# cvjena/mvlm

Hardware: AMD Instinct MI355X
Metric: views/sec (render+CNN+fuse) per mesh, 256x256x96 views (higher is better)
Workload: dtype f32; 1 GPU; configs[2] BU_3DFE-RGB+depth.json: 96 views @ 256x256 of one 99458-triangle textured synthetic face OBJ, 84 landmarks, 4 input channels (RGB+depth), seeded random weights; views_total=96, views_per_gpu=96, landmarks=84, in_channels=4, triangles=99458, selection_method=simple, parallelism=1 GPU, no collective

## Files before the change

### include/mvlm_hip.h

```cpp
#ifndef MVLM_HIP_H
#define MVLM_HIP_H

#include <stddef.h>
#include <stdint.h>

#ifdef __cplusplus
extern "C" {
#endif

typedef struct mvlm_ctx mvlm_ctx;
typedef struct mvlm_mesh mvlm_mesh;
typedef struct mvlm_texture mvlm_texture;

#define MVLM_IMAGE_SIZE 256
#define MVLM_CONV_DESC_INTS 12

enum { MVLM_MODE_QUANTILE = 0, MVLM_MODE_ABSOLUTE = 1 };
enum { MVLM_MAXIMA_SIMPLE = 0, MVLM_MAXIMA_MOMENT = 1 };

int mvlm_ctx_create(int device, mvlm_ctx** out);
void mvlm_ctx_destroy(mvlm_ctx* ctx);
const char* mvlm_last_error(mvlm_ctx* ctx);
int mvlm_set_stream(mvlm_ctx* ctx, void* hip_stream);
int mvlm_synchronize(mvlm_ctx* ctx);
// ... 72 lines not shown
size_t mvlm_cnn_workspace_bytes(mvlm_ctx* ctx, int batch);
int mvlm_cnn_maxima(mvlm_ctx* ctx, const float* images_dev, int n_views, const int32_t* chan_sel_host,
                    float* maxima_dev, void* workspace_dev, size_t workspace_bytes, int batch);
int mvlm_cnn_set_selection(mvlm_ctx* ctx, int method);
int mvlm_cnn_heatmaps(mvlm_ctx* ctx, const float* images_dev, int n_views, const int32_t* chan_sel_host,
                      float* heat_dev, void* workspace_dev, size_t workspace_bytes, int batch);
int mvlm_cnn_set_execution(mvlm_ctx* ctx, int graph_mode, int concurrency);
int mvlm_cnn_set_pairing(mvlm_ctx* ctx, int mode);
int mvlm_cnn_set_winograd(mvlm_ctx* ctx, int mode);
int mvlm_pack_winograd_weights(const float* w9_host, int cin_pad, int cout_pad, float* w12_host);
int mvlm_cnn_set_winograd4(mvlm_ctx* ctx, int mode);
int mvlm_pack_winograd4_weights(const float* w9_host, int cin_pad, int cout_pad, float* w18_host);
int mvlm_cnn_set_winograd4_wide(mvlm_ctx* ctx, int on);
int mvlm_conv_wino4_wide_serves(int ksize, int cin_pad, int cout_pad, int size);
int mvlm_conv_wino4_wide_launches(mvlm_ctx* ctx, int64_t* count, int reset);
int mvlm_cnn_execution_stats(mvlm_ctx* ctx, int64_t* eager_runs, int64_t* graph_captures, int64_t* graph_replays,
                             int64_t* graph_failures);
size_t mvlm_pack_fast_weights(const float* w, int cout, int cin, int cout_pad, int cin_pad, uint16_t* out);
int mvlm_cnn_load_fast(mvlm_ctx* ctx, const uint16_t* blob_host, size_t n_u16, const int64_t* slot_offsets, int n_slots);
int mvlm_cnn_set_precision(mvlm_ctx* ctx, int fast);
int mvlm_conv2d_fast(mvlm_ctx* ctx, const float* x_dev, int batch, int cin, int h, int w, const float* w_host, int cout,
                     const float* bias_host, const float* pre_scale_host, const float* pre_shift_host,
                     const float* post_scale_host, const float* post_shift_host, const float* r_dev, float* y_dev);
size_t mvlm_pack_fast_weights16(const float* w, int cout, int cin, int cout_pad, int cin_pad, uint16_t* out, float* unscale);
int mvlm_cnn_load_fast16(mvlm_ctx* ctx, const uint16_t* blob_host, size_t n_u16, const int64_t* slot_offsets,
                         const float* slot_unscale, int n_slots);
int mvlm_cnn_fast16_overflowed(mvlm_ctx* ctx, int* overflowed);
int mvlm_conv2d_fast16(mvlm_ctx* ctx, const float* x_dev, int batch, int cin, int h, int w, const float* w_host, int cout,
                       const float* bias_host, const float* pre_scale_host, const float* pre_shift_host,
                       const float* post_scale_host, const float* post_shift_host, const float* r_dev, float* y_dev);
// ... 61 lines not shown
```

### mvlm_amd/_lib.py

```python
from __future__ import annotations

import ctypes as C
import os
import subprocess
import threading
from pathlib import Path

_HERE = Path(__file__).resolve().parent
LIB_PATH = Path(os.environ["MVLM_HIP_LIB"]) if os.environ.get("MVLM_HIP_LIB") else _HERE / "lib" / "libmvlm_hip.so"
CSRC = _HERE / "csrc"

c_float_p = C.POINTER(C.c_float)
c_double_p = C.POINTER(C.c_double)
c_int32_p = C.POINTER(C.c_int32)
c_uint8_p = C.POINTER(C.c_uint8)

SIGNATURES = {
    "mvlm_ctx_create": (C.c_int, [C.c_int, C.POINTER(C.c_void_p)]),
    "mvlm_ctx_destroy": (None, [C.c_void_p]),
    "mvlm_last_error": (C.c_char_p, [C.c_void_p]),
    "mvlm_set_stream": (C.c_int, [C.c_void_p, C.c_void_p]),
    "mvlm_synchronize": (C.c_int, [C.c_void_p]),
    "mvlm_build_arch": (C.c_char_p, []),
    "mvlm_obj_read": (C.c_int, [C.c_char_p, C.POINTER(C.c_void_p), C.c_char_p, C.c_int]),
# ... 52 lines not shown
    "mvlm_cnn_workspace_bytes": (C.c_size_t, [C.c_void_p, C.c_int]),
    "mvlm_cnn_maxima": (C.c_int, [C.c_void_p, C.c_void_p, C.c_int, c_int32_p, C.c_void_p, C.c_void_p, C.c_size_t,
                                  C.c_int]),
    "mvlm_cnn_heatmaps": (C.c_int, [C.c_void_p, C.c_void_p, C.c_int, c_int32_p, C.c_void_p, C.c_void_p, C.c_size_t,
                                    C.c_int]),
    "mvlm_cnn_set_execution": (C.c_int, [C.c_void_p, C.c_int, C.c_int]),
    "mvlm_cnn_set_selection": (C.c_int, [C.c_void_p, C.c_int]),
    "mvlm_cnn_set_pairing": (C.c_int, [C.c_void_p, C.c_int]),
    "mvlm_cnn_set_winograd": (C.c_int, [C.c_void_p, C.c_int]),
    "mvlm_pack_winograd_weights": (C.c_int, [c_float_p, C.c_int, C.c_int, c_float_p]),
    "mvlm_cnn_set_winograd4": (C.c_int, [C.c_void_p, C.c_int]),
    "mvlm_pack_winograd4_weights": (C.c_int, [c_float_p, C.c_int, C.c_int, c_float_p]),
    "mvlm_cnn_set_winograd4_wide": (C.c_int, [C.c_void_p, C.c_int]),
    "mvlm_conv_wino4_wide_serves": (C.c_int, [C.c_int, C.c_int, C.c_int, C.c_int]),
    "mvlm_conv_wino4_wide_launches": (C.c_int, [C.c_void_p, C.POINTER(C.c_int64), C.c_int]),
    "mvlm_cnn_execution_stats": (C.c_int, [C.c_void_p, C.POINTER(C.c_int64), C.POINTER(C.c_int64), C.POINTER(C.c_int64),
                                          C.POINTER(C.c_int64)]),
    "mvlm_pack_fast_weights": (C.c_size_t, [c_float_p, C.c_int, C.c_int, C.c_int, C.c_int, C.POINTER(C.c_uint16)]),
    "mvlm_cnn_load_fast": (C.c_int, [C.c_void_p, C.POINTER(C.c_uint16), C.c_size_t, C.POINTER(C.c_int64), C.c_int]),
    "mvlm_cnn_set_precision": (C.c_int, [C.c_void_p, C.c_int]),
    "mvlm_pack_fast_weights16": (C.c_size_t, [c_float_p, C.c_int, C.c_int, C.c_int, C.c_int, C.POINTER(C.c_uint16), c_float_p]),
    "mvlm_cnn_load_fast16": (C.c_int, [C.c_void_p, C.POINTER(C.c_uint16), C.c_size_t, C.POINTER(C.c_int64), c_float_p, C.c_int]),
    "mvlm_cnn_fast16_overflowed": (C.c_int, [C.c_void_p, C.POINTER(C.c_int)]),
    "mvlm_conv2d_fast16": (C.c_int, [C.c_void_p, C.c_void_p, C.c_int, C.c_int, C.c_int, C.c_int, c_float_p, C.c_int, c_float_p,
                                     c_float_p, c_float_p, c_float_p, c_float_p, C.c_void_p, C.c_void_p]),
    "mvlm_conv2d_fast": (C.c_int, [C.c_void_p, C.c_void_p, C.c_int, C.c_int, C.c_int, C.c_int, c_float_p, C.c_int, c_float_p,
                                   c_float_p, c_float_p, c_float_p, c_float_p, C.c_void_p, C.c_void_p]),
    "mvlm_cnn_set_profiling": (C.c_int, [C.c_void_p, C.c_int]),
    "mvlm_cnn_get_profile": (C.c_int, [C.c_void_p, c_int32_p, c_int32_p, c_double_p, c_float_p, C.c_int]),
    "mvlm_conv_variant_name": (C.c_char_p, [C.c_int]),
# ... 140 lines not shown
```

### mvlm_amd/csrc/api.hip

```cpp
#include <atomic>
#include <cstring>

#include <memory>

#include <cmath>

#include "common.h"
#include "raster_points_math.h"
#include "raster_view_math.h"

void* mvlm_ctx::get_scratch(const char* name, size_t bytes) {
    auto& e = scratch[name];
    if (e.second >= bytes && e.first) return e.first;
    if (e.first) {
        hipStreamSynchronize(stream);
        hipFree(e.first);
        e = {nullptr, 0};
    }
    void* p = nullptr;
    const size_t want = bytes + bytes / 4 + 256;
    if (hipMalloc(&p, want) != hipSuccess) return nullptr;
    e = {p, want};
    return p;
}
// ... 19 lines not shown
    *out = ctx;
    return 0;
}

extern "C" void mvlm_ctx_destroy(mvlm_ctx* ctx) {
    if (!ctx) return;
    hipSetDevice(ctx->device);
    hipStreamSynchronize(ctx->stream);
    for (auto& kv : ctx->scratch)
        if (kv.second.first) hipFree(kv.second.first);
    if (ctx->cnn.blob) hipFree(ctx->cnn.blob);
    if (ctx->cnn.fast_blob) hipFree(ctx->cnn.fast_blob);
    if (ctx->cnn.fast16_blob) hipFree(ctx->cnn.fast16_blob);
    for (auto& ww : ctx->cnn.wino)
        if (ww.blob) hipFree(ww.blob);
    if (ctx->cnn.fast16_flag) hipFree(ctx->cnn.fast16_flag);
    if (ctx->switch_event) hipEventDestroy(ctx->switch_event);
    for (int i = 0; i < 2; ++i) {
        if (ctx->kparts_ws[i]) hipFree(ctx->kparts_ws[i]);
        if (ctx->kparts_cnt[i]) hipFree(ctx->kparts_cnt[i]);
    }
    for (auto& e : ctx->mesh_pool) {
        hipFree(e.p);
        if (e.freed) hipEventDestroy(e.freed);
    }
    for (hipEvent_t e : ctx->event_free) hipEventDestroy(e);
    for (int i = 0; i < 2; ++i) {
        if (ctx->upload_stage[i]) hipHostFree(ctx->upload_stage[i]);
        if (ctx->upload_stage_done[i]) hipEventDestroy(ctx->upload_stage_done[i]);
    }
// ... 548 lines not shown
    auto vec = [&](const float* src, int n, int n_pad) -> long {
        if (!src) return -1;
        const size_t off = push(n_pad);
        for (int i = 0; i < n; ++i) blob[off + i] = src[i];
        return long(off);
    };
    long ww_off[MVLM_WINO_FORMS_N];
    for (int f = 0; f < MVLM_WINO_FORMS_N; ++f) {
        const WinoForm& form = mvlm_wino_form(f);
        ww_off[f] = -1;
        if (!form.serves_slot(ksize, cin_pad, cout_pad)) continue;
        ww_off[f] = long(push(size_t(form.slices) * cin_pad * cout_pad));
        form.transform(blob.data() + w_off, cin_pad, cout_pad, blob.data() + ww_off[f]);
    }
    const long b_off = vec(bias_host, cout, cout_pad);
    const long ps_off = vec(pre_scale_host, cin, cin_pad), pt_off = vec(pre_shift_host, cin, cin_pad);
    const long qs_off = vec(post_scale_host, cout, cout_pad), qt_off = vec(post_shift_host, cout, cout_pad);
    auto* d = static_cast<float*>(ctx->get_scratch("conv2d.blob", blob.size() * 4));
    MVLM_REQUIRE(ctx, d, "conv2d: scratch allocation failed");
    MVLM_CHECK_HIP(ctx, hipMemcpy(d, blob.data(), blob.size() * 4, hipMemcpyHostToDevice));
    ConvArgs a;
    a.in = x_dev;
    a.in_ctot = cin;
    a.cin = cin;
    a.cin_pad = cin_pad;
    a.up_in = upsample_in;
    a.B = batch;
    a.H = h;
    a.W = w;
    a.w = d + w_off;
    for (int f = 0; f < MVLM_WINO_FORMS_N; ++f) a.*mvlm_wino_form(f).weights = ww_off[f] < 0 ? nullptr : d + ww_off[f];
    a.cout = cout;
    a.cout_pad = cout_pad;
    a.ksize = ksize;
    a.bias = b_off < 0 ? nullptr : d + b_off;
    a.pre_scale = ps_off < 0 ? nullptr : d + ps_off;
    a.pre_shift = pt_off < 0 ? nullptr : d + pt_off;
    a.post_scale = qs_off < 0 ? nullptr : d + qs_off;
    a.post_shift = qt_off < 0 ? nullptr : d + qt_off;
    a.res1 = r_dev;
    a.res1_ctot = cout;
    a.out = y_dev;
    a.out_ctot = cout;
    if (mvlm_launch_conv(ctx, a, nullptr)) return 1;
    MVLM_CHECK_HIP(ctx, hipStreamSynchronize(ctx->stream));
    return 0;
}

extern "C" int mvlm_conv_bench(mvlm_ctx* ctx, int batch, int cin, int cout, int ksize, int size, int flags, int variant,
                               int iters, float* ms_per_launch, int* variant_used) {
    MVLM_ENTER(ctx);
    MVLM_REQUIRE(ctx, batch > 0 && cin > 0 && cout > 0 && size > 0 && iters > 0 && ms_per_launch, "conv_bench: bad arguments");
    MVLM_REQUIRE(ctx, ksize == 1 || ksize == 3, "conv_bench: kernel size must be 1 or 3");
    const int cin_pad = (ksize == 1 ? (cin + 7) / 8 * 8 : (cin + 3) / 4 * 4), taps = ksize * ksize;
    const bool plain = (flags & 4) && !(flags & (1 | 2 | 8));
    const int cout_pad = (plain && (cout + 15) / 16 * 16 == 80) ? 80 : (plain && ksize == 3 && cout == 84) ? 84 : (cout + 31) / 32 * 32;
    const size_t px = size_t(batch) * size * size;
    const size_t n_w = size_t(ksize == 3 ? 18 : taps) * cin_pad * cout_pad, n_vec = size_t(cin_pad) * 2 + size_t(cout_pad) * 3;
    const size_t n_x = px * cin, n_y = px * cout;
    const size_t total = n_w + n_vec + n_x + 3 * n_y + 64;
    auto* base = static_cast<float*>(ctx->get_scratch("conv_bench", total * sizeof(float)));
    MVLM_REQUIRE(ctx, base, "conv_bench: scratch allocation failed");
    MVLM_CHECK_HIP(ctx, hipMemsetAsync(base, 0, total * sizeof(float), ctx->stream));
    float* w = base;
    float* vec = w + n_w;
    float* x = vec + (n_vec + 3) / 4 * 4;
    float* y = x + (n_x + 3) / 4 * 4;
    float* raw = y + (n_y + 3) / 4 * 4;
    float* res = raw + (n_y + 3) / 4 * 4;
    ConvArgs a;
    a.in = x;
    a.in_ctot = cin;
    a.cin = cin;
    a.cin_pad = cin_pad;
    a.B = batch;
    a.H = a.W = size;
    a.w = w;
    for (int f = 0; f < MVLM_WINO_FORMS_N; ++f)
        if (mvlm_wino_form(f).serves_slot(ksize, cin_pad, cout_pad)) a.*mvlm_wino_form(f).weights = w;
    a.cout = cout;
    a.cout_pad = cout_pad;
    a.ksize = ksize;
    if (flags & 1) {
        a.pre_scale = vec;
        a.pre_shift = vec + cin_pad;
    }
    if (flags & 4) a.bias = vec + 2 * cin_pad;
    if (flags & 8) {
        a.post_scale = vec + 2 * cin_pad + cout_pad;
        a.post_shift = vec + 2 * cin_pad + 2 * cout_pad;
    }
    if (flags & 2) {
        a.res1 = res;
        a.res1_ctot = cout;
// ... 251 lines not shown
```

### mvlm_amd/csrc/cnn_graph.hip

```cpp
#include <cstdlib>

#include "common.h"

namespace {

constexpr long CONCURRENT_MAX_PIXELS_32 = 32l * 32 * 32;

struct Tensor {
    float* p = nullptr;
    int C = 0, S = 0;
    size_t off = 0, elems = 0;
};

struct Block {
    size_t off, size;
    bool free;
    int arena;
    bool deferred;
};

struct Exec {
    mvlm_ctx* ctx;
    CnnState& st;
    int B;
// ... 104 lines not shown
        const int32_t* r = d(slot);
        if (!r[0]) return rc = ctx->fail("cnn: conv slot not present in the packed weights");
        a.in = x.p;
        a.in_ctot = x.C;
        a.in_coff = 0;
        a.cin = r[1];
        a.cout = r[2];
        a.ksize = r[3];
        a.cin_pad = r[4];
        a.cout_pad = r[5];
        a.w = blob(r[6]);
        for (int f = 0; f < MVLM_WINO_FORMS_N; ++f) {
            const CnnState::WinoWeights& ww = st.wino[f];
            a.*mvlm_wino_form(f).weights = (size_t(slot) < ww.off.size() && ww.off[size_t(slot)] >= 0) ? ww.blob + ww.off[size_t(slot)] : nullptr;
        }
        a.bias = blob(r[7]);
        a.pre_scale = blob(r[8]);
        a.pre_shift = blob(r[9]);
        a.post_scale = blob(r[10]);
        a.post_shift = blob(r[11]);
        a.B = B;
        a.H = a.W = S;
        if (x.C != a.cin) return rc = ctx->fail("cnn: channel mismatch between graph and packed weights");
        return 0;
    }
    bool runs_fast(int slot, const ConvArgs& a) const {
        const std::vector<long long>& off = st.fast == 2 ? st.fast16_off : st.fast_off;
        return st.fast && size_t(slot) < off.size() && off[size_t(slot)] >= 0 && mvlm_conv_fast_ok(a, st.fast == 2 ? 2 : 3);
    }
    int prof_begin(hipEvent_t& e0, hipEvent_t& e1) {
// ... 613 lines not shown
        st.fast_blob = nullptr;
    }
    st.fast16_off.clear();
    st.fast16_unscale.clear();
    if (st.fast16_blob) {
        (void)hipFree(st.fast16_blob);
        st.fast16_blob = nullptr;
    }
    for (CnnState::WinoWeights& ww : st.wino) {
        ww.off.clear();
        if (ww.blob) {
            (void)hipFree(ww.blob);
            ww.blob = nullptr;
        }
    }
    st.drop_graphs();
    st.desc.assign(desc_host, desc_host + size_t(n_slots) * MVLM_CONV_DESC_INTS);
    for (int s = 0; s < n_slots; ++s) {
        const int32_t* r = &st.desc[size_t(s) * MVLM_CONV_DESC_INTS];
        if (!r[0]) continue;
        MVLM_REQUIRE(ctx, r[1] > 0 && r[2] > 0 && r[3] >= 1 && r[3] <= 3, "cnn_load: bad conv shape");
        MVLM_REQUIRE(ctx, r[4] % 4 == 0 && r[4] >= r[1] && (r[5] % 16 == 0 || (r[5] == 84 && r[2] == 84 && (r[3] == 3 || r[3] == 2))) && r[5] >= r[2],
                     "cnn_load: bad padding");
        const size_t wsz = size_t(r[3]) * r[3] * r[4] * r[5];
        MVLM_REQUIRE(ctx, r[6] >= 0 && size_t(r[6]) + wsz <= n_floats, "cnn_load: weight offset out of range");
        const int offs[5] = {r[7], r[8], r[9], r[10], r[11]};
        const int lens[5] = {r[5], r[4], r[4], r[5], r[5]};
        for (int k = 0; k < 5; ++k)
            MVLM_REQUIRE(ctx, offs[k] < 0 || size_t(offs[k]) + lens[k] <= n_floats, "cnn_load: vector offset out of range");
    }
// ... 8 lines not shown
        std::vector<float> host;
        ww.off.assign(size_t(n_slots), -1);
        for (int s = 0; s < n_slots; ++s) {
            const int32_t* r = &st.desc[size_t(s) * MVLM_CONV_DESC_INTS];
            if (!r[0] || !form.serves_slot(r[3], r[4], r[5])) continue;
            const size_t off = host.size();
            host.resize(off + size_t(form.slices) * r[4] * r[5]);
            form.transform(blob_host + r[6], r[4], r[5], host.data() + off);
            ww.off[size_t(s)] = (long long)off;
        }
        if (!host.empty()) {
            MVLM_CHECK_HIP(ctx, hipMalloc(&ww.blob, host.size() * sizeof(float)));
            MVLM_CHECK_HIP(ctx, hipMemcpy(ww.blob, host.data(), host.size() * sizeof(float), hipMemcpyHostToDevice));
        }
    }
    st.n_landmarks = n_landmarks;
    st.in_channels = in_channels;
    st.loaded = true;
    return 0;
}

extern "C" size_t mvlm_cnn_workspace_bytes(mvlm_ctx* ctx, int batch) {
    std::lock_guard<std::mutex> lk(ctx->mu);
    if (!ctx->cnn.loaded || batch <= 0) return 0;
    Exec ex(ctx, batch, nullptr, 0, true);
    const int sel4[4] = {0, 0, 0, 0};
    ex.forward(nullptr, sel4, reinterpret_cast<float*>(8), 0, batch, nullptr);
    return ex.high + 256;
}

// ... 56 lines not shown
}

extern "C" int mvlm_cnn_set_winograd(mvlm_ctx* ctx, int mode) {
    return set_winograd_mode(ctx, &mvlm_ctx::conv_winograd, mode, "cnn_set_winograd: 0 never, 1 the measured table (default), 2 every layer a Winograd variant can serve");
}

extern "C" int mvlm_cnn_set_winograd4(mvlm_ctx* ctx, int mode) {
    return set_winograd_mode(ctx, &mvlm_ctx::conv_winograd4, mode, "cnn_set_winograd4: 0 never, 1 the measured table (default), 2 every layer the F(4,3) Winograd tile can serve");
}

extern "C" int mvlm_cnn_set_winograd4_wide(mvlm_ctx* ctx, int on) {
    MVLM_ENTER(ctx);
    MVLM_REQUIRE(ctx, on == 0 || on == 1, "cnn_set_winograd4_wide: 0 the 32 x 16 shape on every launch, 1 the wide shape where the output channels come in 64s (default)");
    if (on != ctx->conv_winograd4_wide) ctx->cnn.drop_graphs();
    ctx->conv_winograd4_wide = on;
    return 0;
}

extern "C" int mvlm_conv_wino4_wide_launches(mvlm_ctx* ctx, int64_t* count, int reset) {
    std::lock_guard<std::mutex> lk(ctx->mu);
    if (count) *count = ctx->conv_wino4_wide_launches;
    if (reset) ctx->conv_wino4_wide_launches = 0;
    return 0;
}

extern "C" int mvlm_cnn_execution_stats(mvlm_ctx* ctx, int64_t* eager_runs, int64_t* graph_captures,
                                        int64_t* graph_replays, int64_t* graph_failures) {
    std::lock_guard<std::mutex> lk(ctx->mu);
    const CnnState& st = ctx->cnn;
    if (eager_runs) *eager_runs = st.eager_runs;
// ... 124 lines not shown
```

### mvlm_amd/csrc/common.h

```cpp
#pragma once
#include <hip/hip_runtime.h>

#include <cstdint>
#include <cstdio>
#include <cstdlib>
#include <map>
#include <mutex>
#include <string>
#include <vector>

#include "../../include/mvlm_hip.h"
#include "jpeg_plan.h"

#define MVLM_CHECK_HIP(ctx, expr)                                                            \
    do {                                                                                     \
        hipError_t _e = (expr);                                                              \
        if (_e != hipSuccess) {                                                              \
            (ctx)->fail(std::string(#expr) + ": " + hipGetErrorString(_e));                  \
            return 1;                                                                        \
        }                                                                                    \
    } while (0)

#define MVLM_ENTER(ctx)                               \
    std::lock_guard<std::mutex> _mvlm_lock((ctx)->mu); \
// ... 24 lines not shown
__host__ __device__ inline bool argmax_better(float ov, int oi, float bv, int bi) {
    const int ok = argmax_key(ov), bk = argmax_key(bv);
    return ok > bk || (ok == bk && oi < bi);
}

struct ConvArgs {
    const float* in = nullptr;
    int in_ctot = 0, in_coff = 0;
    int cin = 0, cin_pad = 0;
    int up_in = 0;
    const float* pre_scale = nullptr;
    const float* pre_shift = nullptr;
    int B = 0, H = 0, W = 0;
    const float* w = nullptr;
    int cout = 0, cout_pad = 0, ksize = 3;
    const float* bias = nullptr;
    const float* post_scale = nullptr;
    const float* post_shift = nullptr;
    const float* res1 = nullptr;
    int res1_ctot = 0, res1_coff = 0;
    const float* res2 = nullptr;
    int res2_ctot = 0, res2_coff = 0;
    float* out_raw = nullptr;
    int raw_ctot = 0, raw_coff = 0;
    float* out = nullptr;
    int out_ctot = 0, out_coff = 0;
    int up_out = 0;
    int sub_y = 0, sub_x = 0;
    int n_par = 1;
    const float* w_par[4] = {nullptr, nullptr, nullptr, nullptr};
// ... 6 lines not shown
    float* kws = nullptr;
    unsigned* kcnt = nullptr;
    float* amax_val = nullptr;
    int* amax_idx = nullptr;
    int amax_parts = 0;
    int amax_part0 = 0;
    float* pool_out = nullptr;
    int pool_ctot = 0, pool_coff = 0;
    float fast_unscale = 1.f;
    int pool_hint = 0;
    unsigned* fast_ovf = nullptr;
    const float* w_wino4 = nullptr;
    unsigned long long* timing = nullptr;
    const float* w_wino = nullptr;
};
static_assert(sizeof(ConvArgs) == 360 && offsetof(ConvArgs, fast_ovf) == 328 && offsetof(ConvArgs, timing) == 344,
              "ConvArgs is passed to the kernels by value: moving a field changes the device code of every convolution kernel");

struct ConvProfileRec {
    int slot, variant;
    double flops;
    hipEvent_t e0, e1;
    short shape[6] = {0, 0, 0, 0, 0, 0};
};

struct ConvOverride {
    short ksize, cin_pad, cout_pad, size, kind;
    int variant;
};
struct ConvKey {
    short ksize, cin_pad, cout_pad, size, kind, batch;
};
// ... 36 lines not shown
    int graph_mode = 1;
    int concurrency = 0;
    int selection = 0;
    int pairing = 1;
    unsigned short* fast_blob = nullptr;
    std::vector<long long> fast_off;
    int fast = 0;
    unsigned short* fast16_blob = nullptr;
    std::vector<long long> fast16_off;
    std::vector<float> fast16_unscale;
    unsigned* fast16_flag = nullptr;
    struct WinoWeights {
        float* blob = nullptr;
        std::vector<long long> off;
    } wino[MVLM_WINO_FORMS_N];
    std::vector<CnnGraphEntry> graphs;
    long graph_replays = 0, graph_captures = 0, eager_runs = 0, graph_failures = 0;
    void drop_graphs() {
        for (CnnGraphEntry& g : graphs)
            if (g.exec) hipGraphExecDestroy(g.exec);
        graphs.clear();
    }
};

struct mvlm_mesh {
    float* verts = nullptr;
    float* uvs = nullptr;
    int32_t* tris = nullptr;
    uint8_t* tex = nullptr;
    uint8_t* colors = nullptr;
// ... 31 lines not shown
    const void* snap_vert_tri = nullptr;
    hipEvent_t switch_event = nullptr;
    bool track_order = false;
    bool order_recorded = false;
    std::mutex mu;
    std::string err;
    CnnState cnn;
    std::map<std::string, std::pair<void*, size_t>> scratch;
    float* kparts_ws[2] = {nullptr, nullptr};
    unsigned* kparts_cnt[2] = {nullptr, nullptr};
    int conv_force_variant = -1;
    int conv_winograd = [] { const char* e = getenv("MVLM_WINOGRAD"); return (e && e[0] >= '0' && e[0] <= '2' && !e[1]) ? e[0] - '0' : 1; }();
    int conv_winograd4 = [] { const char* e = getenv("MVLM_WINOGRAD4"); return (e && e[0] >= '0' && e[0] <= '2' && !e[1]) ? e[0] - '0' : 1; }();
    int conv_winograd4_wide = [] { const char* e = getenv("MVLM_WINOGRAD4_WIDE"); return (e && e[0] >= '0' && e[0] <= '1' && !e[1]) ? e[0] - '0' : 1; }();
    long long conv_wino4_wide_launches = 0;
    std::vector<ConvOverride> conv_overrides;
    unsigned long long conv_attr_mask = 0;
    struct KeyPlaneState {
        const void* ptr = nullptr;
        size_t cap = 0;
    };
    KeyPlaneState raster_keys_clean;
    KeyPlaneState raster_keys4_clean;
    int render_subpixel_bits = 8;
    int render_multisamples = 0;
    int render_shading = 0;
    int* render_overflow_host = nullptr;
    bool points_counting = false;
    std::vector<hipEvent_t> points_events;
    bool points_events_valid = false;
// ... 87 lines not shown
int mvlm_conv_pair_variant(const ConvArgs& a0, const ConvArgs& a1, int mode);
int mvlm_launch_conv_pair(mvlm_ctx* ctx, const ConvArgs& a0, const ConvArgs& a1, int pair_variant);
int mvlm_conv_amax_parts(int H, int W);
const char* mvlm_conv_variant_name_impl(int v);

inline int mvlm_fast_cin_pad(int cin) { return (cin + 15) / 16 * 16; }
inline int mvlm_fast_cout_pad(int cout) { return cout <= 32 ? 32 : (cout + 63) / 64 * 64; }
inline bool mvlm_fast_channels_ok(int cin, int cout) {
    return cin >= 16 && cin <= 256 && cout > 0 && cout * 8 >= mvlm_fast_cout_pad(cout) * 5;
}
bool mvlm_conv_fast_ok(const ConvArgs& a, int splits);
int mvlm_launch_conv_fast(mvlm_ctx* ctx, const ConvArgs& a, const unsigned short* wq_dev, int splits = 3, float unscale = 1.f);
constexpr int MVLM_CONV_VARIANT_WINO4 = 2048;
constexpr int MVLM_CONV_WINO4_ATTR_BIT = 41, MVLM_CONV_WINO4_WIDE_ATTR_BIT = 42, MVLM_CONV_FAST_ATTR_BIT0 = 54;
inline bool mvlm_conv_wino4_wide_shape_ok(int cout_pad, int H) { return cout_pad > 0 && cout_pad % 64 == 0 && H % 16 == 0; }
constexpr int MVLM_CONV_VARIANT_FAST = 62;
constexpr int MVLM_CONV_VARIANT_FAST16 = 61;

int mvlm_launch_landmark_view(mvlm_ctx* ctx, const mvlm_mesh* mesh, const double* rot_host, int n_views, int size,
                              const float* frames_host, const double* landmarks_host, int n_lm, float radius,
                              const uint8_t* lm_rgb_host, uint8_t* out_dev, int32_t* lm_pixels_dev);

int mvlm_launch_ray_view(mvlm_ctx* ctx, const mvlm_mesh* mesh, const double* rot_host, int n_views, int size,
                         const float* frames_host, const double* landmarks_host, int n_lm, float radius, const uint8_t* lm_rgb_host,
                         const double* starts_dev, const double* ends_dev, int n_rays, float ray_radius, const uint8_t* ray_rgb_host,
                         uint8_t* out_dev, int32_t* lm_pixels_dev, int32_t* ray_pixels_dev);

int mvlm_project_partials(mvlm_ctx* ctx, const mvlm_mesh* mesh, const double* pts_dev, int n_points, int* n_chunks_out,
                          const double** part_d_out, const int** part_t_out);

// ... 12 lines not shown
```

### mvlm_amd/csrc/conv_inst_g12.hip

```cpp
#include "conv_kernel.h"
#include "conv_variants.h"

#define X(id, name, ...) \
    int mvlm_conv_launch_##id(mvlm_ctx* ctx, const ConvArgs& a) { return launch_variant<__VA_ARGS__>(ctx, a, id); } \
    int mvlm_conv_pair_launch_##id(mvlm_ctx* ctx, const ConvArgs& a0, const ConvArgs& a1) { return launch_variant_pair<__VA_ARGS__>(ctx, a0, a1, id); }
MVLM_CONV_VARIANTS_G12(X)
#undef X
```

### mvlm_amd/csrc/conv_inst_g3.hip

```cpp
#include "conv_kernel.h"
#include "conv_variants.h"

#define X(id, name, ...) \
    int mvlm_conv_launch_##id(mvlm_ctx* ctx, const ConvArgs& a) { return launch_variant<__VA_ARGS__>(ctx, a, id); } \
    int mvlm_conv_pair_launch_##id(mvlm_ctx* ctx, const ConvArgs& a0, const ConvArgs& a1) { return launch_variant_pair<__VA_ARGS__>(ctx, a0, a1, id); }
MVLM_CONV_VARIANTS_G3(X)
#undef X
```

### mvlm_amd/csrc/conv_inst_q0.hip

```cpp
#include "conv_kernel.h"
#include "conv_variants.h"
#include "conv_wino4_wide_hold.h"

int mvlm_conv_launch_wino4_wide(mvlm_ctx* ctx, const ConvArgs& a);

static bool wide_shape_held(const ConvArgs& a) {
    const int kind = mvlm_conv_kind(a);
    for (int i = 0; i < MVLM_CONV_WINO4_WIDE_HOLD_N; ++i) {
        const ConvWino4WideHold& e = MVLM_CONV_WINO4_WIDE_HOLD[i];
        if (e.cin_pad == a.cin_pad && e.cout_pad == a.cout_pad && e.size == a.H && e.kind == kind) return true;
    }
    return false;
}

int mvlm_conv_launch_wino4(mvlm_ctx* ctx, const ConvArgs& a) {
    if (ctx->conv_winograd4_wide && mvlm_conv_wino4_wide_shape_ok(a.cout_pad, a.H) && !wide_shape_held(a)) return mvlm_conv_launch_wino4_wide(ctx, a);
    return launch_variant<MVLM_CONV_WINO4_CFG>(ctx, a, MVLM_CONV_WINO4_ATTR_BIT);
}
```

### mvlm_amd/csrc/conv_mfma.hip

```cpp
#include <algorithm>
#include <array>
#include <cstdlib>
#include <map>
#include <mutex>
#include <string>
#include <tuple>
#include <vector>

#include "common.h"
#include "conv_kernel.h"
#include "conv_variants.h"
#include "conv_tuned.h"
#include "conv_tuned_net.h"
#include "conv_pair_tuned.h"
#include "conv_tuned_wino.h"
#include "conv_tuned_wino4.h"

#define X(id, name, ...)                                         \
    int mvlm_conv_launch_##id(mvlm_ctx* ctx, const ConvArgs& a); \
    int mvlm_conv_pair_launch_##id(mvlm_ctx* ctx, const ConvArgs& a0, const ConvArgs& a1);
MVLM_CONV_VARIANTS(X)
#undef X
int mvlm_conv_launch_wino4(mvlm_ctx* ctx, const ConvArgs& a);

// ... 321 lines not shown
    MVLM_REQUIRE(ctx, v >= 0, "conv: no kernel variant for this shape");
    const VariantCode d = decode_variant(v);
    const WinoForm* form = d.row && d.row->form >= 0 ? &mvlm_wino_form(d.row->form) : nullptr;
    MVLM_REQUIRE(ctx, !form || a.*form->weights, std::string("conv: a Winograd tile needs the layer's transformed weights (") + form->pack_fn + ")");
    MVLM_REQUIRE(ctx, !a.in2 || v == 0, "conv: a second input tensor needs the 128-channel 8x32 tile (ask mvlm_conv_in2_ok first)");
    MVLM_REQUIRE(ctx, !a.in2 || px / 4 * a.in2_ctot < lim, "conv: second input exceeds 32-bit element offsets");
    MVLM_REQUIRE(ctx, !a.pool_out || mvlm_conv_variant_can_pool(v), "conv: this shape's kernel variant cannot emit the pooled tensor");
    MVLM_REQUIRE(ctx, !a.pool_out || px / 4 * a.pool_ctot < lim, "conv: pooled output exceeds 32-bit element offsets");
    MVLM_REQUIRE(ctx, !form || !a.amax_val || a.out || a.pool_out, "conv: a Winograd tile has no fused argmax, and no other output is requested");
    MVLM_REQUIRE(ctx, a.out || a.pool_out || a.amax_val, "conv: no output requested");
    if (variant_out) *variant_out = v;
    MVLM_REQUIRE(ctx, d.kparts > 0, "conv: unknown kernel variant");
    ConvArgs b = a;
    b.kparts = d.kparts;
    if (form) b.w = a.*form->weights;
    return d.row ? d.row->launch(ctx, b) : ctx->fail("conv: unreachable variant");
}


extern "C" int mvlm_conv_variant_serves(int variant, int ksize, int cin_pad, int cout_pad, int size, int kind) {
    const VariantCode d = decode_variant(variant);
    const ConvVariantInfo* t = d.row;
    if (!t || ksize != 3 || kind < 0 || kind > 2 || !tile_fits(*t, ksize, cin_pad, cout_pad, size, size)) return 0;
    const int parts = d.kparts;
    const bool residual_block_tile = !t->TAIL16 && t->COUT_T != 96;
    const bool bn_fits = t->form < 0 || cin_pad <= t->BN_MAXC;
    const bool parts_ok = parts == 1 || (t->SPLITK && t->PIX_T == 32 && cin_pad % (parts * t->CK) == 0);
    return residual_block_tile && bn_fits && parts_ok;
}

extern "C" int mvlm_conv_wino4_wide_serves(int ksize, int cin_pad, int cout_pad, int size) {
// ... 43 lines not shown
            const double g0 = w9[size_t(kx) * n + i], g1 = w9[size_t(3 + kx) * n + i], g2 = w9[size_t(6 + kx) * n + i];
            w18[size_t(kx) * n + i] = float(g0);
            w18[size_t(3 + kx) * n + i] = float(0.0 - (g0 + g1 + g2) / 3.0);
            w18[size_t(6 + kx) * n + i] = float((g0 - g1 + g2) / 3.0);
            w18[size_t(9 + kx) * n + i] = float((g0 + 2.0 * g1 + 4.0 * g2) / 15.0);
            w18[size_t(12 + kx) * n + i] = float((-16.0 * g0 + 8.0 * g1 - 4.0 * g2) / 15.0);
            w18[size_t(15 + kx) * n + i] = float(g2);
        }
}

extern "C" int mvlm_pack_winograd4_weights(const float* w9_host, int cin_pad, int cout_pad, float* w18_host) {
    if (!w9_host || !w18_host || cin_pad <= 0 || cout_pad <= 0) return 1;
    mvlm_winograd4_transform(w9_host, cin_pad, cout_pad, w18_host);
    return 0;
}
```

Baseline: 1278 views/s.

## Route 80/84-channel conv layers to Winograd F(4,3) with zero-padded weights

Adds a path that pads the Winograd-4 transformed weights and bias of layers whose output channels are not a multiple of 32 (80 or 84) up to the next multiple of 32. Those layers can then run on the existing Winograd-4 kernel instead of the direct 80/84-row tiles. A tuned table turns this on by default for 256-in, 128x128 plain layers at batch 96 or more. It does extra multiply work on the padded output columns and adds a second weight blob to device memory.

```diff
diff --git a/include/mvlm_hip.h b/include/mvlm_hip.h
--- a/include/mvlm_hip.h
+++ b/include/mvlm_hip.h
@@ -110,6 +110,11 @@
 int mvlm_cnn_set_winograd4_wide(mvlm_ctx* ctx, int on);
 int mvlm_conv_wino4_wide_serves(int ksize, int cin_pad, int cout_pad, int size);
 int mvlm_conv_wino4_wide_launches(mvlm_ctx* ctx, int64_t* count, int reset);
+int mvlm_cnn_set_winograd4_padded(mvlm_ctx* ctx, int mode);
+int mvlm_conv_wino4_padded_launches(mvlm_ctx* ctx, int64_t* count, int reset);
+int mvlm_conv_wino4_padded_stride(int cout_pad);
+int mvlm_pack_winograd4_weights_padded(const float* w9_host, const float* bias_host, int cin_pad, int cout_pad, float* w18_pad_host,
+                                       float* bias_pad_host);
 int mvlm_cnn_execution_stats(mvlm_ctx* ctx, int64_t* eager_runs, int64_t* graph_captures, int64_t* graph_replays,
                              int64_t* graph_failures);
 size_t mvlm_pack_fast_weights(const float* w, int cout, int cin, int cout_pad, int cin_pad, uint16_t* out);
diff --git a/mvlm_amd/_lib.py b/mvlm_amd/_lib.py
--- a/mvlm_amd/_lib.py
+++ b/mvlm_amd/_lib.py
@@ -90,6 +90,10 @@
     "mvlm_cnn_set_winograd4_wide": (C.c_int, [C.c_void_p, C.c_int]),
     "mvlm_conv_wino4_wide_serves": (C.c_int, [C.c_int, C.c_int, C.c_int, C.c_int]),
     "mvlm_conv_wino4_wide_launches": (C.c_int, [C.c_void_p, C.POINTER(C.c_int64), C.c_int]),
+    "mvlm_cnn_set_winograd4_padded": (C.c_int, [C.c_void_p, C.c_int]),
+    "mvlm_conv_wino4_padded_launches": (C.c_int, [C.c_void_p, C.POINTER(C.c_int64), C.c_int]),
+    "mvlm_conv_wino4_padded_stride": (C.c_int, [C.c_int]),
+    "mvlm_pack_winograd4_weights_padded": (C.c_int, [c_float_p, c_float_p, C.c_int, C.c_int, c_float_p, c_float_p]),
     "mvlm_cnn_execution_stats": (C.c_int, [C.c_void_p, C.POINTER(C.c_int64), C.POINTER(C.c_int64), C.POINTER(C.c_int64),
                                           C.POINTER(C.c_int64)]),
     "mvlm_pack_fast_weights": (C.c_size_t, [c_float_p, C.c_int, C.c_int, C.c_int, C.c_int, C.POINTER(C.c_uint16)]),
diff --git a/mvlm_amd/csrc/api.hip b/mvlm_amd/csrc/api.hip
--- a/mvlm_amd/csrc/api.hip
+++ b/mvlm_amd/csrc/api.hip
@@ -57,6 +57,7 @@
     if (ctx->cnn.fast16_blob) hipFree(ctx->cnn.fast16_blob);
     for (auto& ww : ctx->cnn.wino)
         if (ww.blob) hipFree(ww.blob);
+    if (ctx->cnn.wino4_pad_blob) hipFree(ctx->cnn.wino4_pad_blob);
     if (ctx->cnn.fast16_flag) hipFree(ctx->cnn.fast16_flag);
     if (ctx->switch_event) hipEventDestroy(ctx->switch_event);
     for (int i = 0; i < 2; ++i) {
@@ -635,6 +636,14 @@
         form.transform(blob.data() + w_off, cin_pad, cout_pad, blob.data() + ww_off[f]);
     }
     const long b_off = vec(bias_host, cout, cout_pad);
+    long wp_off = -1, bp_off = -1;
+    if (mvlm_conv_wino4_pad_serves_slot(ksize, cin_pad, cout_pad)) {
+        const int P = mvlm_conv_wino4_padded_cout(cout_pad);
+        wp_off = long(push(size_t(18) * cin_pad * P));
+        if (b_off >= 0) bp_off = long(push(size_t(P)));
+        mvlm_winograd4_pack_padded(blob.data() + w_off, b_off < 0 ? nullptr : blob.data() + b_off, cin_pad, cout_pad, blob.data() + wp_off,
+                                   bp_off < 0 ? nullptr : blob.data() + bp_off);
+    }
     const long ps_off = vec(pre_scale_host, cin, cin_pad), pt_off = vec(pre_shift_host, cin, cin_pad);
     const long qs_off = vec(post_scale_host, cout, cout_pad), qt_off = vec(post_shift_host, cout, cout_pad);
     auto* d = static_cast<float*>(ctx->get_scratch("conv2d.blob", blob.size() * 4));
@@ -663,6 +672,8 @@
     a.res1_ctot = cout;
     a.out = y_dev;
     a.out_ctot = cout;
+    ctx->conv_wino4_pads[0] = {wp_off < 0 ? nullptr : d + wp_off, bp_off < 0 ? nullptr : d + bp_off};
+    a.wino4_pad = wp_off < 0 ? 0 : 1;
     if (mvlm_launch_conv(ctx, a, nullptr)) return 1;
     MVLM_CHECK_HIP(ctx, hipStreamSynchronize(ctx->stream));
     return 0;
@@ -677,7 +688,7 @@
     const bool plain = (flags & 4) && !(flags & (1 | 2 | 8));
     const int cout_pad = (plain && (cout + 15) / 16 * 16 == 80) ? 80 : (plain && ksize == 3 && cout == 84) ? 84 : (cout + 31) / 32 * 32;
     const size_t px = size_t(batch) * size * size;
-    const size_t n_w = size_t(ksize == 3 ? 18 : taps) * cin_pad * cout_pad, n_vec = size_t(cin_pad) * 2 + size_t(cout_pad) * 3;
+    const size_t n_w = size_t(ksize == 3 ? 18 : taps) * cin_pad * mvlm_conv_wino4_padded_cout(cout_pad), n_vec = size_t(cin_pad) * 2 + size_t(cout_pad) * 3;
     const size_t n_x = px * cin, n_y = px * cout;
     const size_t total = n_w + n_vec + n_x + 3 * n_y + 64;
     auto* base = static_cast<float*>(ctx->get_scratch("conv_bench", total * sizeof(float)));
@@ -699,6 +710,9 @@
     a.w = w;
     for (int f = 0; f < MVLM_WINO_FORMS_N; ++f)
         if (mvlm_wino_form(f).serves_slot(ksize, cin_pad, cout_pad)) a.*mvlm_wino_form(f).weights = w;
+    const bool padded = mvlm_conv_wino4_pad_serves_slot(ksize, cin_pad, cout_pad);
+    ctx->conv_wino4_pads[0] = padded ? ConvWino4Pad{w, vec + 2 * cin_pad} : ConvWino4Pad{};
+    a.wino4_pad = padded ? 1 : 0;
     a.cout = cout;
     a.cout_pad = cout_pad;
     a.ksize = ksize;
diff --git a/mvlm_amd/csrc/cnn_graph.hip b/mvlm_amd/csrc/cnn_graph.hip
--- a/mvlm_amd/csrc/cnn_graph.hip
+++ b/mvlm_amd/csrc/cnn_graph.hip
@@ -1,3 +1,4 @@
+#include <array>
 #include <cstdlib>
 
 #include "common.h"
@@ -142,6 +143,7 @@
             const CnnState::WinoWeights& ww = st.wino[f];
             a.*mvlm_wino_form(f).weights = (size_t(slot) < ww.off.size() && ww.off[size_t(slot)] >= 0) ? ww.blob + ww.off[size_t(slot)] : nullptr;
         }
+        a.wino4_pad = size_t(slot) < st.wino4_pad_id.size() ? st.wino4_pad_id[size_t(slot)] : 0;
         a.bias = blob(r[7]);
         a.pre_scale = blob(r[8]);
         a.pre_shift = blob(r[9]);
@@ -785,6 +787,12 @@
             ww.blob = nullptr;
         }
     }
+    st.wino4_pad_id.clear();
+    ctx->conv_wino4_pads.resize(1);
+    if (st.wino4_pad_blob) {
+        (void)hipFree(st.wino4_pad_blob);
+        st.wino4_pad_blob = nullptr;
+    }
     st.drop_graphs();
     st.desc.assign(desc_host, desc_host + size_t(n_slots) * MVLM_CONV_DESC_INTS);
     for (int s = 0; s < n_slots; ++s) {
@@ -823,6 +831,29 @@
             MVLM_CHECK_HIP(ctx, hipMemcpy(ww.blob, host.data(), host.size() * sizeof(float), hipMemcpyHostToDevice));
         }
     }
+    {
+        std::vector<float> host;
+        std::vector<std::array<long long, 3>> made;
+        for (int s = 0; s < n_slots; ++s) {
+            const int32_t* r = &st.desc[size_t(s) * MVLM_CONV_DESC_INTS];
+            if (!r[0] || !mvlm_conv_wino4_pad_serves_slot(r[3], r[4], r[5])) continue;
+            const int P = mvlm_conv_wino4_padded_cout(r[5]);
+            const size_t w_off = host.size(), b_off = w_off + size_t(18) * r[4] * P;
+            host.resize(b_off + (r[7] >= 0 ? P : 0));
+            mvlm_winograd4_pack_padded(blob_host + r[6], r[7] >= 0 ? blob_host + r[7] : nullptr, r[4], r[5], host.data() + w_off,
+                                       r[7] >= 0 ? host.data() + b_off : nullptr);
+            made.push_back({s, (long long)w_off, r[7] >= 0 ? (long long)b_off : -1});
+        }
+        if (!host.empty()) {
+            MVLM_CHECK_HIP(ctx, hipMalloc(&st.wino4_pad_blob, host.size() * sizeof(float)));
+            MVLM_CHECK_HIP(ctx, hipMemcpy(st.wino4_pad_blob, host.data(), host.size() * sizeof(float), hipMemcpyHostToDevice));
+            st.wino4_pad_id.assign(size_t(n_slots), 0);
+            for (const auto& m : made) {
+                ctx->conv_wino4_pads.push_back({st.wino4_pad_blob + m[1], m[2] < 0 ? nullptr : st.wino4_pad_blob + m[2]});
+                st.wino4_pad_id[size_t(m[0])] = int(ctx->conv_wino4_pads.size());
+            }
+        }
+    }
     st.n_landmarks = n_landmarks;
     st.in_channels = in_channels;
     st.loaded = true;
@@ -909,6 +940,18 @@
     MVLM_REQUIRE(ctx, on == 0 || on == 1, "cnn_set_winograd4_wide: 0 the 32 x 16 shape on every launch, 1 the wide shape where the output channels come in 64s (default)");
     if (on != ctx->conv_winograd4_wide) ctx->cnn.drop_graphs();
     ctx->conv_winograd4_wide = on;
+    return 0;
+}
+
+extern "C" int mvlm_cnn_set_winograd4_padded(mvlm_ctx* ctx, int mode) {
+    return set_winograd_mode(ctx, &mvlm_ctx::conv_winograd4_padded, mode,
+                             "cnn_set_winograd4_padded: 0 never, 1 the measured table (default), 2 every eligible launch of the 80- and 84-row tiles");
+}
+
+extern "C" int mvlm_conv_wino4_padded_launches(mvlm_ctx* ctx, int64_t* count, int reset) {
+    std::lock_guard<std::mutex> lk(ctx->mu);
+    if (count) *count = ctx->conv_wino4_padded_launches;
+    if (reset) ctx->conv_wino4_padded_launches = 0;
     return 0;
 }
 
diff --git a/mvlm_amd/csrc/common.h b/mvlm_amd/csrc/common.h
--- a/mvlm_amd/csrc/common.h
+++ b/mvlm_amd/csrc/common.h
@@ -62,6 +62,7 @@
     int B = 0, H = 0, W = 0;
     const float* w = nullptr;
     int cout = 0, cout_pad = 0, ksize = 3;
+    int wino4_pad = 0;
     const float* bias = nullptr;
     const float* post_scale = nullptr;
     const float* post_shift = nullptr;
@@ -98,8 +99,14 @@
     unsigned long long* timing = nullptr;
     const float* w_wino = nullptr;
 };
-static_assert(sizeof(ConvArgs) == 360 && offsetof(ConvArgs, fast_ovf) == 328 && offsetof(ConvArgs, timing) == 344,
+static_assert(sizeof(ConvArgs) == 360 && offsetof(ConvArgs, wino4_pad) == 84 && offsetof(ConvArgs, bias) == 88 && offsetof(ConvArgs, fast_ovf) == 328 &&
+                  offsetof(ConvArgs, timing) == 344,
               "ConvArgs is passed to the kernels by value: moving a field changes the device code of every convolution kernel");
+
+struct ConvWino4Pad {
+    const float* w = nullptr;
+    const float* bias = nullptr;
+};
 
 struct ConvProfileRec {
     int slot, variant;
@@ -166,6 +173,8 @@
         float* blob = nullptr;
         std::vector<long long> off;
     } wino[MVLM_WINO_FORMS_N];
+    float* wino4_pad_blob = nullptr;
+    std::vector<int> wino4_pad_id;
     std::vector<CnnGraphEntry> graphs;
     long graph_replays = 0, graph_captures = 0, eager_runs = 0, graph_failures = 0;
     void drop_graphs() {
@@ -227,6 +236,10 @@
     int conv_winograd4 = [] { const char* e = getenv("MVLM_WINOGRAD4"); return (e && e[0] >= '0' && e[0] <= '2' && !e[1]) ? e[0] - '0' : 1; }();
     int conv_winograd4_wide = [] { const char* e = getenv("MVLM_WINOGRAD4_WIDE"); return (e && e[0] >= '0' && e[0] <= '1' && !e[1]) ? e[0] - '0' : 1; }();
     long long conv_wino4_wide_launches = 0;
+    int conv_winograd4_padded = [] { const char* e = getenv("MVLM_WINOGRAD4_PADDED"); return (e && e[0] >= '0' && e[0] <= '2' && !e[1]) ? e[0] - '0' : 1; }();
+    long long conv_wino4_padded_launches = 0;
+    std::vector<ConvWino4Pad> conv_wino4_pads = std::vector<ConvWino4Pad>(1);
+    int conv_launch_ran_as = -1;
     std::vector<ConvOverride> conv_overrides;
     unsigned long long conv_attr_mask = 0;
     struct KeyPlaneState {
@@ -344,6 +357,11 @@
 constexpr int MVLM_CONV_VARIANT_WINO4 = 2048;
 constexpr int MVLM_CONV_WINO4_ATTR_BIT = 41, MVLM_CONV_WINO4_WIDE_ATTR_BIT = 42, MVLM_CONV_FAST_ATTR_BIT0 = 54;
 inline bool mvlm_conv_wino4_wide_shape_ok(int cout_pad, int H) { return cout_pad > 0 && cout_pad % 64 == 0 && H % 16 == 0; }
+inline int mvlm_conv_wino4_padded_cout(int cout_pad) { return (cout_pad + 31) / 32 * 32; }
+inline bool mvlm_conv_wino4_pad_serves_slot(int ksize, int cin_pad, int cout_pad) {
+    return cout_pad > 0 && cout_pad % 32 != 0 && mvlm_conv_wino4_serves_slot(ksize, cin_pad, mvlm_conv_wino4_padded_cout(cout_pad));
+}
+void mvlm_winograd4_pack_padded(const float* w9, const float* bias, int cin_pad, int cout_pad, float* w18_pad, float* bias_pad);
 constexpr int MVLM_CONV_VARIANT_FAST = 62;
 constexpr int MVLM_CONV_VARIANT_FAST16 = 61;
 
diff --git a/mvlm_amd/csrc/conv_inst_g12.hip b/mvlm_amd/csrc/conv_inst_g12.hip
--- a/mvlm_amd/csrc/conv_inst_g12.hip
+++ b/mvlm_amd/csrc/conv_inst_g12.hip
@@ -1,8 +1,11 @@
 #include "conv_kernel.h"
 #include "conv_variants.h"
 
+bool mvlm_conv_wino4_padded_takes(const mvlm_ctx* ctx, const ConvArgs& a);
+int mvlm_conv_launch_wino4_padded(mvlm_ctx* ctx, const ConvArgs& a);
+
 #define X(id, name, ...) \
-    int mvlm_conv_launch_##id(mvlm_ctx* ctx, const ConvArgs& a) { return launch_variant<__VA_ARGS__>(ctx, a, id); } \
+    int mvlm_conv_launch_##id(mvlm_ctx* ctx, const ConvArgs& a) { return mvlm_conv_wino4_padded_takes(ctx, a) ? mvlm_conv_launch_wino4_padded(ctx, a) : launch_variant<__VA_ARGS__>(ctx, a, id); } \
     int mvlm_conv_pair_launch_##id(mvlm_ctx* ctx, const ConvArgs& a0, const ConvArgs& a1) { return launch_variant_pair<__VA_ARGS__>(ctx, a0, a1, id); }
 MVLM_CONV_VARIANTS_G12(X)
 #undef X
diff --git a/mvlm_amd/csrc/conv_inst_g3.hip b/mvlm_amd/csrc/conv_inst_g3.hip
--- a/mvlm_amd/csrc/conv_inst_g3.hip
+++ b/mvlm_amd/csrc/conv_inst_g3.hip
@@ -1,8 +1,11 @@
 #include "conv_kernel.h"
 #include "conv_variants.h"
 
+bool mvlm_conv_wino4_padded_takes(const mvlm_ctx* ctx, const ConvArgs& a);
+int mvlm_conv_launch_wino4_padded(mvlm_ctx* ctx, const ConvArgs& a);
+
 #define X(id, name, ...) \
-    int mvlm_conv_launch_##id(mvlm_ctx* ctx, const ConvArgs& a) { return launch_variant<__VA_ARGS__>(ctx, a, id); } \
+    int mvlm_conv_launch_##id(mvlm_ctx* ctx, const ConvArgs& a) { return mvlm_conv_wino4_padded_takes(ctx, a) ? mvlm_conv_launch_wino4_padded(ctx, a) : launch_variant<__VA_ARGS__>(ctx, a, id); } \
     int mvlm_conv_pair_launch_##id(mvlm_ctx* ctx, const ConvArgs& a0, const ConvArgs& a1) { return launch_variant_pair<__VA_ARGS__>(ctx, a0, a1, id); }
 MVLM_CONV_VARIANTS_G3(X)
 #undef X
diff --git a/mvlm_amd/csrc/conv_inst_q0.hip b/mvlm_amd/csrc/conv_inst_q0.hip
--- a/mvlm_amd/csrc/conv_inst_q0.hip
+++ b/mvlm_amd/csrc/conv_inst_q0.hip
@@ -1,6 +1,7 @@
 #include "conv_kernel.h"
 #include "conv_variants.h"
 #include "conv_wino4_wide_hold.h"
+#include "conv_tuned_wino4_pad.h"
 
 int mvlm_conv_launch_wino4_wide(mvlm_ctx* ctx, const ConvArgs& a);
 
@@ -17,3 +18,31 @@
     if (ctx->conv_winograd4_wide && mvlm_conv_wino4_wide_shape_ok(a.cout_pad, a.H) && !wide_shape_held(a)) return mvlm_conv_launch_wino4_wide(ctx, a);
     return launch_variant<MVLM_CONV_WINO4_CFG>(ctx, a, MVLM_CONV_WINO4_ATTR_BIT);
 }
+
+bool mvlm_conv_wino4_padded_takes(const mvlm_ctx* ctx, const ConvArgs& a) {
+    if (a.wino4_pad <= 0 || size_t(a.wino4_pad) > ctx->conv_wino4_pads.size() || !ctx->conv_wino4_pads[size_t(a.wino4_pad) - 1].w) return false;
+    if (a.ksize != 3 || a.up_in || a.in2 || a.amax_val || a.res1 || a.res2 || a.post_scale || a.out_raw || a.pool_out || a.up_out || !a.out || a.n_par != 1 ||
+        a.kparts > 1 || a.H != a.W || a.H % 16 != 0 || a.cin_pad > 256 || (a.bias && !ctx->conv_wino4_pads[size_t(a.wino4_pad) - 1].bias))
+        return false;
+    if (ctx->conv_force_variant >= 0) return false;
+    if (ctx->conv_winograd == 0 || ctx->conv_winograd4 == 0 || ctx->conv_winograd4_padded == 0) return false;
+    if (ctx->conv_winograd4_padded == 2) return true;
+    const int kind = mvlm_conv_kind(a);
+    for (int i = 0; i < MVLM_CONV_TUNED_WINO4_PAD_N; ++i) {
+        const ConvTunedWino4Pad& e = MVLM_CONV_TUNED_WINO4_PAD[i];
+        if (e.cin_pad == a.cin_pad && e.cout_pad == a.cout_pad && e.size == a.H && e.kind == kind && a.B >= e.min_batch) return true;
+    }
+    return false;
+}
+
+int mvlm_conv_launch_wino4_padded(mvlm_ctx* ctx, const ConvArgs& a) {
+    const ConvWino4Pad& p = ctx->conv_wino4_pads[size_t(a.wino4_pad) - 1];
+    ConvArgs b = a;
+    b.w = p.w;
+    b.bias = a.bias ? p.bias : nullptr;
+    b.cout_pad = mvlm_conv_wino4_padded_cout(a.cout_pad);
+    if (launch_variant<MVLM_CONV_WINO4_CFG>(ctx, b, MVLM_CONV_WINO4_ATTR_BIT)) return 1;
+    ++ctx->conv_wino4_padded_launches;
+    ctx->conv_launch_ran_as = MVLM_CONV_VARIANT_WINO4;
+    return 0;
+}
diff --git a/mvlm_amd/csrc/conv_mfma.hip b/mvlm_amd/csrc/conv_mfma.hip
--- a/mvlm_amd/csrc/conv_mfma.hip
+++ b/mvlm_amd/csrc/conv_mfma.hip
@@ -359,7 +359,11 @@
     ConvArgs b = a;
     b.kparts = d.kparts;
     if (form) b.w = a.*form->weights;
-    return d.row ? d.row->launch(ctx, b) : ctx->fail("conv: unreachable variant");
+    if (!d.row) return ctx->fail("conv: unreachable variant");
+    ctx->conv_launch_ran_as = -1;
+    const int rc = d.row->launch(ctx, b);
+    if (variant_out && ctx->conv_launch_ran_as >= 0) *variant_out = ctx->conv_launch_ran_as;
+    return rc;
 }
 
 
@@ -433,3 +437,27 @@
     mvlm_winograd4_transform(w9_host, cin_pad, cout_pad, w18_host);
     return 0;
 }
+
+void mvlm_winograd4_pack_padded(const float* w9, const float* bias, int cin_pad, int cout_pad, float* w18_pad, float* bias_pad) {
+    const int P = mvlm_conv_wino4_padded_cout(cout_pad);
+    const size_t rows = size_t(18) * cin_pad;
+    std::vector<float> w18(rows * cout_pad);
+    mvlm_winograd4_transform(w9, cin_pad, cout_pad, w18.data());
+    for (size_t r = 0; r < rows; ++r) {
+        std::copy(w18.begin() + r * cout_pad, w18.begin() + (r + 1) * cout_pad, w18_pad + r * P);
+        std::fill(w18_pad + r * P + cout_pad, w18_pad + (r + 1) * P, 0.f);
+    }
+    if (bias && bias_pad) {
+        std::copy(bias, bias + cout_pad, bias_pad);
+        std::fill(bias_pad + cout_pad, bias_pad + P, 0.f);
+    }
+}
+
+extern "C" int mvlm_conv_wino4_padded_stride(int cout_pad) { return cout_pad > 0 ? mvlm_conv_wino4_padded_cout(cout_pad) : 0; }
+
+extern "C" int mvlm_pack_winograd4_weights_padded(const float* w9_host, const float* bias_host, int cin_pad, int cout_pad, float* w18_pad_host,
+                                                  float* bias_pad_host) {
+    if (!w9_host || !w18_pad_host || cin_pad <= 0 || cout_pad <= 0 || (bias_host && !bias_pad_host)) return 1;
+    mvlm_winograd4_pack_padded(w9_host, bias_host, cin_pad, cout_pad, w18_pad_host, bias_pad_host);
+    return 0;
+}
diff --git a/mvlm_amd/csrc/conv_tuned_wino4_pad.h b/mvlm_amd/csrc/conv_tuned_wino4_pad.h
--- /dev/null
+++ b/mvlm_amd/csrc/conv_tuned_wino4_pad.h
@@ -0,0 +1,12 @@
+#ifndef MVLM_CONV_TUNED_WINO4_PAD_H
+#define MVLM_CONV_TUNED_WINO4_PAD_H
+struct ConvTunedWino4Pad {
+    short cin_pad, cout_pad, size, kind, min_batch;
+};
+static const ConvTunedWino4Pad MVLM_CONV_TUNED_WINO4_PAD[] = {
+    {256, 80, 128, 0, 96},
+    {256, 84, 128, 0, 96},
+    {0, 0, 0, 0, 0},
+};
+static const int MVLM_CONV_TUNED_WINO4_PAD_N = 2;
+#endif
```

After: 1346 views/s, median of 6. 1.05x the previous value.
